# Mingqj/DFU3D

Hardware: AMD Instinct MI355X
Metric: pseudo-box frames/sec (34k pts, 6 cams) (higher is better)
Workload: dtype f64; 1 GPU; configs[1] with depth back-projection on (dense): 64 synthetic frames/GPU/step, 34720-pt sweep, 6 cams x 1600x900 depth + 8 instance masks (one bit-packed 1-byte word per pixel), 30-40 objects/scene; views_per_launch_chunk=192, streams=2, parallelism=frames sharded x1

## Files before the change

dfu3d_amd/csrc/common.hpp:

```cpp
#pragma once
#include <hip/hip_runtime.h>
#include <stdint.h>

#include <stddef.h>
#include <string.h>
#include "dfu3d.h"
#include "dbg.hpp"

#define DFU3D_WAVE 64

struct ViewCalib {
  float M43[12];
  float P2[12];
  float cu, cv, fu, fv, tx, ty;
  float Minv[12];
  float pad[6];
};
static_assert(sizeof(ViewCalib) == DFU3D_CALIB_FLOATS * 4, "calib record");

__device__ __forceinline__ int lane_id() { return threadIdx.x & 63; }

__device__ __forceinline__ int wave_rank(bool flag, int &wave_total) {
  const unsigned long long m = __ballot(flag);
  wave_total = __popcll(m);
  return __popcll(m & ((1ull << lane_id()) - 1ull));
}

template <int NW>
__device__ __forceinline__ int block_rank(bool flag, int *s_w, int &block_total) {
  int wt;
  const int r = wave_rank(flag, wt);
  const int w = threadIdx.x >> 6;
// ... 327 lines not shown
```

dfu3d_amd/csrc/fit_stage.hip:

```cpp
#include "common.hpp"

namespace {
__device__ __forceinline__ int rl_i(int v, int l) { return __builtin_amdgcn_readlane(v, l); }
__device__ __forceinline__ double rl_d(double v, int l) {
  return __hiloint2double(__builtin_amdgcn_readlane(__double2hiint(v), l), __builtin_amdgcn_readlane(__double2loint(v), l));
}

constexpr int CT = 512;
constexpr int GRP = 32;
constexpr int BLK = 32;
constexpr int PAIR_SMALL = 32;
constexpr int GU = 4;
constexpr int SMALL_N = 4096;
constexpr int LARGE_N = 61440;
constexpr int LARGE_GRP = LARGE_N / GRP;
constexpr int GRID_NC_SMALL = 4096;
constexpr int GRID_NC_LARGE = 12288;

struct ParI {
  int *p;
  bool global;
  __device__ __forceinline__ int load(int i) const {
    return __hip_atomic_load(p + i, __ATOMIC_RELAXED, __HIP_MEMORY_SCOPE_AGENT);
  }
// ... 376 lines not shown
  while (true) {
    a = cell_find(par, a);
    b = cell_find(par, b);
    if (a == b) return;
    if (a < b) { const int t = a; a = b; b = t; }
    const int old = atomicMin(par + a, b);
    if (old == a) return;
    a = old;
  }
}

constexpr int CL_CLASSES = 3, CL_TOP = 8192;
template <int NC, int NC_MIN, int TCT>
__global__ __launch_bounds__(TCT, (NC <= GRID_NC_SMALL ? 8 : 4)) void k_range_cluster_grid(
    const double *__restrict__ px, const double *__restrict__ py,
    const long long *__restrict__ seg_base, const int *__restrict__ seg_cnt, double R0,
    double Rd, int *__restrict__ label, double *__restrict__ sx, double *__restrict__ sy,
    int *__restrict__ perm_all, long long pool_cap, int n_lo, int n_hi) {
  __shared__ int s_end[NC];
  __shared__ int s_par[NC];
  __shared__ int s_min[NC];
  __shared__ double s_red[5 * (TCT / 64)];
  __shared__ int s_w[TCT / 64];
  constexpr int NCLS = CL_CLASSES;
  const int S_ = (int)(gridDim.x / (unsigned)NCLS);
  const int cls = (int)(blockIdx.x / (unsigned)S_);
  const int s = (int)(blockIdx.x - (unsigned)cls * (unsigned)S_);
  const int n = seg_cnt[s];
  if (n <= n_lo || n > n_hi) return;
  {
    int mine = NCLS - 1;
#pragma unroll
    for (int k = NCLS - 2; k >= 0; k--) if (n > (CL_TOP >> k)) mine = k;
    if (mine != cls) return;
  }
  const long long base = seg_base[s];
  const double *X = px + base, *Y = py + base;
  double *SX = sx + base, *SY = sy + base;
  int *perm = perm_all + base;
  int *mark = perm_all + 2 * pool_cap + base;
  if (NC_MIN > 0 && *mark) return;
  const GridGeom<NC> G = grid_geometry<NC, TCT>(X, Y, n, R0, Rd, s_red);
  if (threadIdx.x == 0 && (NC_MIN == 0 || G.ok)) *mark = G.ok ? 1 : 0;
  if (!G.ok) return;
  const int ncell = G.ncell;
  for (int c = threadIdx.x; c < ncell; c += TCT) { s_end[c] = 0; s_par[c] = c; s_min[c] = 0x7FFFFFFF; }
// ... 223 lines not shown
#pragma unroll
    for (int u = 0; u < GU; u++) {
      const int i = i0 + u * TCT;
      xs[u] = (i < n) ? SX[i] : 0.0; ys[u] = (i < n) ? SY[i] : 0.0; pm[u] = (i < n) ? perm[i] : 0;
    }
#pragma unroll
    for (int u = 0; u < GU; u++)
      if (i0 + u * TCT < n) glabel[pm[u]] = s_min[cell_find(s_par, grid_cell(G, xs[u], ys[u]))];
  }
}

__global__ __launch_bounds__(CT) void k_range_cluster_fallback(
    const double *__restrict__ px, const double *__restrict__ py,
    const long long *__restrict__ seg_base, const int *__restrict__ seg_cnt, double R0,
    double Rd, int *__restrict__ label, double *__restrict__ sx, double *__restrict__ sy,
    int *__restrict__ si, long long pool_cap) {
  __shared__ __attribute__((aligned(16))) unsigned short s_parent[LARGE_N];
  __shared__ int s_summ[LARGE_GRP];
  __shared__ float4 s_box[LARGE_GRP];
  __shared__ int s_summ2[LARGE_GRP / BLK];
  __shared__ float4 s_box2[LARGE_GRP / BLK];
  __shared__ double s_red[4 * (CT / 64)];
  __shared__ int s_w[CT / 64];
  static_assert(sizeof(int) * SMALL_N <= sizeof(unsigned short) * LARGE_N && SMALL_N / GRP <= LARGE_GRP, "the small form fits");
  const int s = blockIdx.x;
  const int n = seg_cnt[s];
  if (n == 0) return;
  const long long base = seg_base[s];
  if (si[2 * pool_cap + base]) return;
  if (n <= SMALL_N) {
    cell_sort<SMALL_N>(px + base, py + base, n, (int *)s_parent, s_red, s_w, sx + base, sy + base, si + base);
    ParI par{(int *)s_parent, false};
    cluster_body<ParI, SMALL_N / GRP>(par, s_summ, s_box, s_summ2, s_box2, s_red, sx + base, sy + base,
                                      n, R0, Rd, si + base, si + pool_cap + base, label + base);
    return;
  }
  cell_sort<LARGE_N / 2>(px + base, py + base, n, (int *)s_parent, s_red, s_w, sx + base, sy + base,
                         si + base);
  if (n <= LARGE_N) {
    ParH par{s_parent};
    cluster_body<ParH, LARGE_GRP>(par, s_summ, s_box, s_summ2, s_box2, s_red, sx + base, sy + base,
                                  n, R0, Rd, si + base, si + pool_cap + base, label + base);
  } else {
    ParI par{si + 2 * pool_cap + base, true};
    cluster_body<ParI, LARGE_GRP>(par, s_summ, s_box, s_summ2, s_box2, s_red, sx + base, sy + base,
                                  n, R0, Rd, si + base, si + pool_cap + base, label + base);
// ... 95 lines not shown

__device__ __forceinline__ int rank_in(const int *roots, int nk, int L) {
  int lo = 0, hi = nk - 1;
  while (lo < hi) {
    const int mid = (lo + hi) >> 1;
    if (roots[mid] < L) lo = mid + 1; else hi = mid;
  }
  return (roots[lo] == L) ? lo : -1;
}

constexpr int GGU = 4;
__global__ __launch_bounds__(FT) void k_fit_gather(
    const double *__restrict__ px, const double *__restrict__ py,
    const double *__restrict__ pz, const int *__restrict__ label,
    const long long *__restrict__ seg_base, const int *__restrict__ seg_cnt,
    double *__restrict__ gsx, double *__restrict__ gsy, int *__restrict__ sroot,
    uint32_t *__restrict__ status, double *__restrict__ fit_ws, int cap_rows, int cap_big) {
  __shared__ int s_roots[GK];
  __shared__ int s_cnt[FW][GK];
  __shared__ int s_tot[GK], s_off[GK];
  __shared__ double s_red[FW];
  __shared__ int s_w[FW];
  __shared__ int s_q0, s_total;
  const int S_ = (int)(gridDim.x / 3u);
  const int cls = (int)(blockIdx.x / (unsigned)S_);
  const int s = (int)(blockIdx.x - (unsigned)cls * (unsigned)S_);
  const int n = seg_cnt[s];
  if (n == 0) return;
  if (cls != (n > 16384 ? 0 : (n > 8192 ? 1 : 2))) return;
  const long long base = seg_base[s];
  const int wave = threadIdx.x >> 6, lane = lane_id();
  const FitWs W = fit_ws_view(fit_ws, cap_rows, cap_big);

  const int R = (((n + FW - 1) / FW) + 63) & ~63;
  const int r0 = min(n, wave * R), r1 = min(n, r0 + R);
  double zm = -INFINITY;
  int mine = 0;
  for (int c = r0; c < r1; c += 64 * GGU) {
    int L[GGU];
    double zz[GGU];
#pragma unroll
    for (int u = 0; u < GGU; u++) {
      const int i = c + u * 64 + lane;
      L[u] = (i < r1) ? label[base + i] : -1;
      zz[u] = (i < r1) ? pz[base + i] : -INFINITY;
    }
// ... 319 lines not shown
  e.wave_reduce();
  if (lane_id() == 0) { s_ext[wave][0] = e.a0; s_ext[wave][1] = e.a1; s_ext[wave][2] = e.b0; s_ext[wave][3] = e.b1; }
  __syncthreads();
  if (threadIdx.x == 0) {
    double c1min = s_ext[0][0], c1max = s_ext[0][1], c2min = s_ext[0][2], c2max = s_ext[0][3];
    for (int w = 1; w < FW; w++) {
      c1min = fmin(c1min, s_ext[w][0]); c1max = fmax(c1max, s_ext[w][1]);
      c2min = fmin(c2min, s_ext[w][2]); c2max = fmax(c2max, s_ext[w][3]);
    }
    const int s = (int)dsc[0], kc = (int)dsc[1], root = (int)dsc[2];
    const int v = s / max_inst, jinst = s - v * max_inst;
    emit_box(thb, sin_s, cos_s, c1min, c1max, c2min, c2max, dsc[5], s, v, jinst, kc, root, m, calib, inst_class,
             inst_is_car, inst_box, inst_score, car_aspect_max, cap_rows, rows, n_rows, status);
  }
}

__global__ __launch_bounds__(256) void k_fit_tiny(
    const double *__restrict__ gsx, const double *__restrict__ gsy, int max_inst,
    const ViewCalib *__restrict__ calib, const int *__restrict__ inst_class,
    const int *__restrict__ inst_is_car, const float *__restrict__ inst_box,
    const float *__restrict__ inst_score, int n_theta, double dtheta, double car_aspect_max,
    int cap_rows, double *__restrict__ rows, int *__restrict__ n_rows,
    uint32_t *__restrict__ status, double *__restrict__ fit_ws, int cap_big) {
  const FitWs W = fit_ws_view(fit_ws, cap_rows, cap_big);
  const int nq = min(W.counters[0], W.cap_q);
  const int lane = lane_id();
  const int gw = (blockIdx.x * 256 + threadIdx.x) >> 6, nw = (gridDim.x * 256) >> 6;
  for (int e = gw; e < nq; e += nw) {
    const double *d = W.dsc + (size_t)8 * e;
    const int m = (int)d[3];
    if (m > 64) continue;
    const long long P = (long long)d[4];
    const double x = (lane < m) ? gsx[P + lane] : 0.0, y = (lane < m) ? gsy[P + lane] : 0.0;
    const LanePoints pts{x, y, m};
    constexpr int TH_PER_LANE = MAXTH / 64;
    double c1t[TH_PER_LANE], magmax = 0.0, top = -INFINITY;
#pragma unroll
    for (int k = 0; k < TH_PER_LANE; k++) {
      const int th = lane + 64 * k;
      c1t[k] = -INFINITY;
      if (64 * k >= n_theta) continue;
      const double theta = (double)th * dtheta;
      const double ct = cos(theta), st = sin(theta);
      Extent ext;
      ext.clear();
      pts.each([&](double xj, double yj) {
// ... 181 lines not shown
    }
#pragma unroll
    for (int h = 0; h < BIGC_HPW; h++) {
      A[h].wave_reduce();
      double mag;
      const double cst = A[h].cost(mag);
      if (lane == 0 && th[h] < n_theta) {
        W.big_cost[(size_t)c * MAXTH + th[h]] = cst;
        if (mag > 0.0) atomicMax((unsigned long long *)(W.dsc + (size_t)8 * W.big_list[c] + 7), (unsigned long long)__double_as_longlong(mag));
      }
    }
  }
}

__global__ __launch_bounds__(FT) void k_fit_big_box(
    const double *__restrict__ gsx, const double *__restrict__ gsy, int max_inst,
    const ViewCalib *__restrict__ calib, const int *__restrict__ inst_class,
    const int *__restrict__ inst_is_car, const float *__restrict__ inst_box,
    const float *__restrict__ inst_score, int n_theta, double dtheta, double car_aspect_max,
    int cap_rows, double *__restrict__ rows, int *__restrict__ n_rows,
    uint32_t *__restrict__ status, double *__restrict__ fit_ws, int cap_big) {
  __shared__ double s_ext[FW][4];
  __shared__ double s_ct[MAXTH], s_st[MAXTH];
  const FitWs W = fit_ws_view(fit_ws, cap_rows, cap_big);
  const int nbig = min(W.counters[1], cap_big);
  fill_heading_table(s_ct, s_st, dtheta);
  for (int c = blockIdx.x; c < nbig; c += gridDim.x) {
    __syncthreads();
    const double *dsc = W.dsc + (size_t)8 * W.big_list[c];
    const int m = (int)dsc[3];
    const double *mx = gsx + (long long)dsc[4], *my = gsy + (long long)dsc[4];
    const int best = wave_pick_heading(W.big_cost + (size_t)c * MAXTH, n_theta, dsc[7], mx, my, m, s_ct, s_st);
    fit_finish(mx, my, m, dsc, best, dtheta, s_ext, max_inst, calib, inst_class, inst_is_car, inst_box, inst_score,
               car_aspect_max, cap_rows, rows, n_rows, status);
  }
}

}

extern "C" int dfu3d_range_cluster(const double *px, const double *py, const int64_t *seg_base,
                                   const int32_t *seg_cnt, int32_t S, double R0, double Rd,
                                   int32_t *label, double *sx, double *sy, int32_t *si,
                                   int64_t pool_cap, void *stream) {
  DFU3D_CLEAR_STALE_ERROR();
  if (!px || !py || !seg_base || !seg_cnt || !label || !sx || !sy || !si) return DFU3D_EINVAL;
  if (S <= 0 || pool_cap <= 0 || !(R0 > 0.0) || !(Rd >= 0.0)) return DFU3D_EINVAL;
// ... 84 lines not shown
```

dfu3d_amd/csrc/lidar_stage.hip:

```cpp
#include "common.hpp"

namespace {

constexpr int NT = 512;
constexpr int NW = NT / 64;

constexpr int FOV_PW = 1024;
__global__ __launch_bounds__(NT) void k_fov_filter(
    const float4 *__restrict__ pts, const int *__restrict__ pt_off,
    const int *__restrict__ view_frame, const ViewCalib *__restrict__ calib,
    float fovH, float fovW, int capN, int *__restrict__ fov_idx,
    int *__restrict__ n_fov) {
  __shared__ int s_w[NW];
  const int v = blockIdx.x;
  const int f = view_frame[v];
  const int p0 = pt_off[f];
  const int n = pt_off[f + 1] - p0;
  const ViewCalib c = calib[v];
  const int wave = threadIdx.x >> 6, lane = lane_id();
  int running = 0;
  for (int base = 0; base < n; base += NW * FOV_PW) {
    const int w0 = base + wave * FOV_PW;
    unsigned long long flags[FOV_PW / 64];
    int mine = 0;
#pragma unroll
    for (int k = 0; k < FOV_PW / 64; k++) {
      const int i = w0 + k * 64 + lane;
      bool ok = false;
      if (i < n) {
        const float4 p = pts[p0 + i];
        float r[3], u, w, d;
        lidar_to_rect_f32(c.M43, p.x, p.y, p.z, r);
        rect_to_img_f32(c.P2, r, u, w, d);
        ok = (u >= 0.0f) && (u < fovW) && (w >= 0.0f) && (w < fovH) && (d >= 0.0f);
      }
      flags[k] = __ballot(ok);
// ... 147 lines not shown
  return t;
}
__device__ __forceinline__ int block_sum_i(int v, int *s_red) {
  v = wave_sum_i(v);
  const int w = threadIdx.x >> 6;
  __syncthreads();
  if (lane_id() == 0) s_red[w] = v;
  __syncthreads();
  int t = 0;
#pragma unroll
  for (int i = 0; i < NW; i++) t += s_red[i];
  return t;
}

constexpr int RB = 8;
constexpr int RS_LDS = 3072;

__global__ __launch_bounds__(NT) void k_plane_ransac(
    const float4 *__restrict__ pts, const int *__restrict__ pt_off,
    const int *__restrict__ view_frame, const int *__restrict__ fov_idx,
    const int *__restrict__ n_fov, int capN, float max_hs, float xy_range,
    int trials, unsigned long long seed, const long long *__restrict__ key,
    int *__restrict__ cand_idx, double *__restrict__ plane) {
  __shared__ int s_w[NW];
  __shared__ int s_hist[256];
  __shared__ unsigned long long s_sel[3];
  __shared__ double s_red[NW];
  __shared__ int s_redi[NW];
  __shared__ double s_model[RB][3];
  __shared__ int s_valid[RB], s_tot[RB], s_cnt[NW][RB];
  __shared__ float4 s_pt[RS_LDS];
  const int v = blockIdx.x;
  const int p0 = pt_off[view_frame[v]];
  const int nf = n_fov[v];
  const int *fidx = fov_idx + (size_t)v * capN;
  int *cidx = cand_idx + (size_t)v * capN;
  int n = 0;
  for (int base = 0; base < nf; base += NT) {
    const int t = base + threadIdx.x;
    bool ok = false;
    int pi = 0;
    if (t < nf) {
      pi = fidx[t];
      const float4 p = pts[p0 + pi];
      ok = (p.z < max_hs) && (p.x > -xy_range) && (p.x < xy_range) &&
           (p.y > -xy_range) && (p.y < xy_range);
// ... 120 lines not shown
    const double det2 = sxx * syy - sxy * sxy;
    const double ref = fmax(sxx * syy, 1e-300);
    if (det2 > 1e-12 * ref) {
      ca = (sxz * syy - syz * sxy) / det2;
      cb = (syz * sxx - sxz * sxy) / det2;
      cc = (mz - ca * mx) - cb * my;
    }
    const double norm = sqrt((ca * ca + cb * cb) + 1.0);
    out[0] = -(ca / norm);
    out[1] = -(cb / norm);
    out[2] = 1.0 / norm;
    out[3] = -(cc / norm);
  }
}

__global__ __launch_bounds__(NT) void k_project_rows(
    const float4 *__restrict__ pts, const int *__restrict__ pt_off,
    const int *__restrict__ view_frame, const ViewCalib *__restrict__ calib,
    const double *__restrict__ plane, const int *__restrict__ fov_idx,
    const int *__restrict__ n_fov, int capN, float boundH, float boundW, int W,
    double plane_offset, float xy_range, int *__restrict__ ag_pt,
    int *__restrict__ ib_pix, int *__restrict__ n_ag, int *__restrict__ Kout) {
  __shared__ int s_w[NW];
  const int v = blockIdx.x;
  const int p0 = pt_off[view_frame[v]];
  const int nf = n_fov[v];
  const ViewCalib c = calib[v];
  const double pl0 = plane[v * 4 + 0], pl1 = plane[v * 4 + 1], pl2 = plane[v * 4 + 2],
               pl3 = plane[v * 4 + 3];
  const double pn = sqrt((pl0 * pl0 + pl1 * pl1) + pl2 * pl2);
  const int *fidx = fov_idx + (size_t)v * capN;
  int nag = 0, nib = 0;
  for (int base = 0; base < nf; base += NT) {
    const int t = base + threadIdx.x;
    bool ag = false, ib = false;
    int pi = 0, pix = 0;
    if (t < nf) {
      pi = fidx[t];
      const float4 p = pts[p0 + pi];
      double d = (((double)p.x * pl0 + (double)p.y * pl1) + (double)p.z * pl2) + pl3;
      d = d / pn;
      const bool below = d < plane_offset;
      const bool inr = (p.x < xy_range) && (p.x > -xy_range) && (p.y < xy_range) && (p.y > -xy_range);
      ag = !(below && inr);
      if (ag) {
        float r[3], u, w, dep;
// ... 153 lines not shown
```

dfu3d_amd/csrc/segment_stage.hip:

```cpp
#include "common.hpp"

namespace {

constexpr int QT = 256;
constexpr int PT = 1024;

__device__ __forceinline__ uint32_t shadow_word(int seg, double radius) {
  float rf = (float)radius;
  if (radius > 0.0 && (double)rf > radius) rf = __uint_as_float(__float_as_uint(rf) - 1u);
  uint32_t hi = __float_as_uint(rf) >> 16;
  if (radius > 0.0 && hi == 0u) hi = 1u;
  if (radius != radius) hi = 0x7FC0u;
  return ((uint32_t)seg << 16) | hi;
}


constexpr int SEG_WI = 256, SEG_STEPS = SEG_WI / 64;
constexpr int SEG_WPB = 4;
constexpr int SEG_GX = 128;
static_assert(DFU3D_MAX_INST == 32, "one lane per instance, instance bits in one 32-bit word; k_seg_scan: 32 x 32 threads");
inline int seg_ranges(int cap_item) { return (cap_item + SEG_WI - 1) / SEG_WI; }

__device__ __forceinline__ uint32_t wave_or_u32(uint32_t x) { return wave_or_u32_dpp(x); }

// ... 12 lines not shown
  return mine;
}

__global__ __launch_bounds__(SEG_WPB * 64) void k_seg_count(const uint32_t *__restrict__ bits,
                                                            const int *__restrict__ n_item, int cap_item, int NR,
                                                            int *__restrict__ range_cnt) {
  const int v = blockIdx.y;
  const int lane = lane_id();
  const int wave = __builtin_amdgcn_readfirstlane((int)(threadIdx.x >> 6));
  const int n = min(n_item[v], cap_item);
  const int nr = (n + SEG_WI - 1) / SEG_WI;
  for (int r = blockIdx.x * SEG_WPB + wave; r < nr; r += gridDim.x * SEG_WPB) {
    uint32_t b[SEG_STEPS], wany[SEG_STEPS];
#pragma unroll
    for (int k = 0; k < SEG_STEPS; k++) {
      const int t = r * SEG_WI + k * 64 + lane;
      b[k] = (t < n) ? bits[(size_t)v * cap_item + t] : 0u;
    }
    const int mine = wave_instance_counts(b, wany);
    if (lane < DFU3D_MAX_INST) range_cnt[((size_t)v * NR + r) * DFU3D_MAX_INST + lane] = mine;
  }
}

struct SegSide {
  const int *n_item;
  int cap_item, NR;
  int *range_cnt, *cnt;
};
__global__ __launch_bounds__(1024) void k_seg_scan(SegSide A, SegSide B, int max_inst) {
  __shared__ int s_g[32][DFU3D_MAX_INST + 1];
  const SegSide X = blockIdx.y ? B : A;
  const int v = blockIdx.x;
  const int j = threadIdx.x & (DFU3D_MAX_INST - 1), g = threadIdx.x / DFU3D_MAX_INST;
  const int n = min(X.n_item[v], X.cap_item);
  const int nr = (n + SEG_WI - 1) / SEG_WI;
  const int per = (nr + 31) / 32;
  int *col = X.range_cnt + (size_t)v * X.NR * DFU3D_MAX_INST + j;
  const int r0 = g * per, r1 = min(r0 + per, nr);
  int sum = 0;
  for (int r = r0; r < r1; r++) sum += col[(size_t)r * DFU3D_MAX_INST];
  s_g[g][j] = sum;
  __syncthreads();
  int run = 0, tot = 0;
#pragma unroll 8
  for (int q = 0; q < 32; q++) {
    const int c = s_g[q][j];
    run += (q < g) ? c : 0;
    tot += c;
  }
  for (int r = r0; r < r1; r++) {
    const int c = col[(size_t)r * DFU3D_MAX_INST];
    col[(size_t)r * DFU3D_MAX_INST] = run;
    run += c;
  }
  if (g == 0 && j < max_inst) X.cnt[v * max_inst + j] = tot;
}

struct JointSegs {
  long long *base;
  int *cnt;
  double *rad;
  const double *rad_a, *rad_b;
};

__global__ __launch_bounds__(1024) void k_seg_alloc(int S, int *__restrict__ cnt_a,
                                                    int *__restrict__ cnt_b,
                                                    long long *__restrict__ base_a,
                                                    long long *__restrict__ base_b,
                                                    long long pool_cap,
                                                    long long *__restrict__ cursor,
                                                    uint32_t *__restrict__ status, JointSegs J) {
  __shared__ int s_w[16];
  __shared__ long long s_end;
  long long running = *cursor;
  bool over = false;
  if (threadIdx.x == 0) s_end = -1;
  __syncthreads();
  for (int b0 = 0; b0 < S; b0 += 1024) {
    const int s = b0 + threadIdx.x;
    const int ca = (s < S) ? cnt_a[s] : 0, cb = (s < S) ? cnt_b[s] : 0;
    int tot;
    const int ex = block_excl_scan<16>(ca + cb, s_w, tot);
    if (s < S) {
      const long long b = running + ex;
      if (b + ca + cb > pool_cap) {
        cnt_a[s] = 0;
        cnt_b[s] = 0;
        base_a[s] = 0;
        base_b[s] = 0;
        if (ca + cb > 0) {
          over = true;
          atomicMin((unsigned long long *)&s_end, (unsigned long long)b);
        }
      } else {
        base_a[s] = b;
        base_b[s] = b + ca;
      }
      if (J.base) {
        J.base[s] = base_a[s]; J.base[S + s] = base_b[s];
        J.cnt[s] = cnt_a[s]; J.cnt[S + s] = cnt_b[s];
        J.rad[s] = J.rad_a[s]; J.rad[S + s] = J.rad_b[s];
      }
    }
    running += tot;
  }
  if (over) atomicOr(status, DFU3D_ST_POOL_OVERFLOW);
  __syncthreads();
// ... 45 lines not shown
      for (uint32_t w = wany[k]; w; w &= w - 1u) {
        const int j = __ffs((int)w) - 1;
        const bool has = (b[k] >> j) & 1u;
        const unsigned long long m = __ballot(has);
        const long long start = (long long)(((unsigned long long)(uint32_t)__builtin_amdgcn_readlane((int)(woff >> 32), j) << 32) |
                                            (uint32_t)__builtin_amdgcn_readlane((int)(woff & 0xFFFFFFFFll), j));
        const uint32_t swj = (uint32_t)__builtin_amdgcn_readlane((int)sw, j);
        if (has) {
          const long long d = start + __popcll(m & ((1ull << lane) - 1ull));
          px[d] = x[k];
          py[d] = y[k];
          pz[d] = z[k];
          if (pq)
            pq[d] = make_float4((float)x[k], (float)y[k], (float)z[k], __uint_as_float(swj));
        }
        if (lane == j) woff += __popcll(m);
      }
    }
  }
}

template <class F>
__device__ __forceinline__ void tile_scan(int S, F tiles, int *__restrict__ tile_off) {
  __shared__ int s_w[16];
  const int total = block_scan_range<1024, 1, int, int>(S, tiles, [&](int s, int ex) { tile_off[s] = ex; }, s_w);
  if (threadIdx.x == 0) tile_off[S] = total;
}

__global__ __launch_bounds__(1024) void k_tile_scan(int S, const int *__restrict__ cnt,
                                                    int *__restrict__ tile_off, int qt) {
  tile_scan(S, [&](int s) { return (cnt[s] + qt - 1) / qt; }, tile_off);
}

__device__ __forceinline__ int find_segment(const int *tile_off, int S, int t) {
  int lo = 0, hi = S;
  while (hi - lo > 1) {
    const int mid = (lo + hi) >> 1;
    if (tile_off[mid] <= t) lo = mid; else hi = mid;
  }
  return lo;
}

constexpr int RFB = 256;
constexpr int RF_IT = 8;
constexpr int RF_WG = RFB * RF_IT;
constexpr int RF_STRIDE = 8;
constexpr int RF_OCC = 8;
constexpr int RF_GRID = 8192;
constexpr int RF_WLIST = 128;
constexpr int RF_WIN = 16;
constexpr int RF_PLDS = RF_WLIST + 2 * RF_WIN;
constexpr uint32_t RF_NOSEG = 0xFFFFu;
constexpr int BOX_FLOATS = 16;
// ... 428 lines not shown
    cnt += __popcll(__ballot(hit));
  }
  if (big) {
#pragma unroll
    for (int u = 0; u < RF_UL; u++) {
      const bool b = lane + 64 < un[u];
      o[u] = b ? W.uent[ur[u] * RF_WLIST + 64 + lane] : make_float4(0.f, 0.f, 0.f, 0.f);
      op[u] = b ? W.upos[ur[u] * RF_WLIST + 64 + lane] : 0u;
    }
#pragma unroll
    for (int u = 0; u < RF_UL; u++) {
      const bool hit = (op[u] & RF_INCOH) && __float_as_uint(o[u].w) == Q.wq && rf_within(Q, o[u], (long long)(op[u] & ~RF_INCOH), px, py, pz);
      cnt += __popcll(__ballot(hit));
    }
  }
  return cnt;
}

__global__ __launch_bounds__(256, 5) void k_rf_resolve(
    const double *__restrict__ px, const double *__restrict__ py, const double *__restrict__ pz,
    const float4 *__restrict__ pq, const long long *__restrict__ n_used_ptr, long long n_max,
    const long long *__restrict__ seg_base, const int *__restrict__ seg_cnt, const double *__restrict__ radius,
    int nb, int S, RfScratch W) {
  long long n_used = n_max;
  if (n_used_ptr) { const long long u = *n_used_ptr; n_used = u < n_max ? u : n_max; }
  const int wave = (blockIdx.x * 256 + threadIdx.x) >> 6;
  const int nwaves = (gridDim.x * 256) >> 6;
  const int lane = lane_id();
  const int q_incl = wave_incl_scan((int)min((long long)max(W.queue[16 * lane], 0), W.qcap));
  const int nq = __builtin_amdgcn_readlane(q_incl, 63);
  int *lq_tab = W.work + RF_WORK_LQ, *items = W.work + RF_WORK_ITEMS;
  for (int e = wave; e < nq; e += nwaves) {
    const int part = __popcll(__ballot(q_incl <= e));
    const int before = part ? __builtin_amdgcn_readlane(q_incl, part - 1) : 0;
    RfQuery Q;
    if (!rf_load_query(Q, W.queue[RF_QHDR + part * W.qcap + (e - before)], n_max, pq, px, py, pz, seg_base, seg_cnt, radius, S)) continue;
    const int n = (int)(Q.end - Q.base);
    int cnt = 0, n_items = 0, lq = -1;
    if (n <= RF_DIRECT) {
      const long long c_lo = Q.base >> 6, c_hi = (Q.end - 1) >> 6;
      for (long long c0 = c_lo; c0 <= c_hi && cnt <= nb; c0 += RF_SC) {
        float4 o[RF_SC];
#pragma unroll
        for (int u = 0; u < RF_SC; u++) o[u] = pq[((c0 + u) << 6) + lane];
#pragma unroll
        for (int u = 0; u < RF_SC; u++) {
// ... 120 lines not shown
      if ((int)(old >> 32) + 1 == total) W.flags[Q.i] = ((int)(old & 0xFFFFFFFFull) + hits > nb) ? 1 : 0;
    }
  }
}


__global__ __launch_bounds__(QT) void k_shadow_build(
    const double *__restrict__ px, const double *__restrict__ py, const double *__restrict__ pz,
    const long long *__restrict__ seg_base, const int *__restrict__ seg_cnt,
    const double *__restrict__ radius, int S, const int *__restrict__ tile_off, float4 *__restrict__ pq) {
  const int ntile = tile_off[S];
  for (int t = blockIdx.x; t < ntile; t += gridDim.x) {
    const int s = find_segment(tile_off, S, t);
    const int q = (t - tile_off[s]) * QT + threadIdx.x;
    if (q >= seg_cnt[s]) continue;
    const long long i = seg_base[s] + q;
    pq[i] = make_float4((float)px[i], (float)py[i], (float)pz[i], __uint_as_float(shadow_word(s, radius[s])));
  }
}

constexpr int BT_BIG = 1024, BH_HEADS_BIG = 8192, BH_MAX_BIG = 4096;
constexpr int BT_SMALL = 256, BH_HEADS_SMALL = 2048, BH_MAX_SMALL = 1024;

__global__ __launch_bounds__(1024) void k_tile_scan_class(int S, const int *__restrict__ cnt, const int *__restrict__ cnt_a,
                                                          int lo, int hi, int *__restrict__ tile_off, int qt) {
  tile_scan(S, [&](int s) {
    const int na = cnt_a[s];
    return (na > lo && na <= hi) ? (cnt[s] + qt - 1) / qt : 0;
  }, tile_off);
}

__device__ __forceinline__ uint32_t sad_u32(uint32_t a, uint32_t b) {
  uint32_t r;
  asm("v_sad_u32 %0, %1, %2, 0" : "=v"(r) : "v"(a), "v"(b));
  return r;
}
__device__ __forceinline__ uint32_t bh_hash(uint32_t ix, uint32_t iy, uint32_t iz) {
  uint32_t h = __umul24(ix, 0x9E3779u) ^ __umul24(iy, 0x85EBCBu) ^ __umul24(iz, 0xC2B2AFu);
  h ^= h >> 15;
  h ^= h >> 7;
  return h;
}

constexpr int BALL_TPW = 1;
template <int BT, int BH_MAX, int BH_HEADS>
__global__ __launch_bounds__(BT) void k_ball_flags(
    const double *__restrict__ px, const double *__restrict__ py,
    const double *__restrict__ pz, const long long *__restrict__ base_a,
// ... 161 lines not shown
          double d = dx * dx;
          d += dy * dy;
          d += dz * dz;
          if (d < T) { found = true; break; }
        }
        if (!found) s_pending = 1;
      }
      __syncthreads();
      if (!s_pending && any_kept) break;
    }
    if (valid && any_kept) flags[bq + q] = found ? 1 : 0;
  }
}


constexpr int CPT = 1024;
constexpr int CPE = 2;
__global__ __launch_bounds__(CPT) void k_seg_compact(
    double *__restrict__ px, double *__restrict__ py, double *__restrict__ pz,
    long long *__restrict__ seg_base, int *__restrict__ seg_cnt,
    const uint8_t *__restrict__ flags, const long long *__restrict__ dst_after_base,
    int *__restrict__ dst_after_cnt, int compact_front) {
  __shared__ int s_w[CPT / 64];
  const int s = blockIdx.x;
  const int n = seg_cnt[s];
  const long long src = seg_base[s];
  const int front_all = dst_after_base ? dst_after_cnt[s] : 0;
  const int front = (compact_front && dst_after_base) ? front_all : 0;
  const long long src_f = dst_after_base ? dst_after_base[s] : 0;
  const long long dst = dst_after_base ? src_f + (front_all - front) : src;
  const int n_all = front + n;
  if (n_all == 0) {
    if (dst_after_base && threadIdx.x == 0) seg_base[s] = dst;
    return;
  }
  int running = 0, kept_front = 0;
  for (int t0 = 0; t0 < n_all; t0 += CPT * CPE) {
    const int i0 = t0 + threadIdx.x * CPE;
    bool f[CPE];
    double x[CPE], y[CPE], z[CPE];
    int mine = 0;
#pragma unroll
    for (int k = 0; k < CPE; k++) {
      const int i = i0 + k;
      const long long g = (i < front) ? src_f + i : src + (i - front);
      f[k] = (i < n_all) && flags[g];
// ... 249 lines not shown
    double *pz, int64_t *base_a, int32_t *cnt_a, int64_t *base_b, int32_t *cnt_b,
    uint32_t *status, const double *rad_a, const double *rad_b, void *shadow, int64_t *base_ab,
    int32_t *cnt_ab, double *rad_ab, int32_t *chunk_cnt, void *stream) {
  DFU3D_CLEAR_STALE_ERROR();
  if (!a_bits || !a_x || !a_y || !a_z || !a_n || !b_bits || !b_x || !b_y || !b_z || !b_n ||
      !pool_cursor || !px || !py || !pz || !base_a || !cnt_a || !base_b || !cnt_b || !status || !chunk_cnt)
    return DFU3D_EINVAL;
  if (V <= 0 || max_inst <= 0 || a_cap <= 0 || b_cap <= 0 || pool_cap <= 0) return DFU3D_EINVAL;
  if (max_inst > DFU3D_MAX_INST) return DFU3D_ERANGE;
  if ((shadow || base_ab) && (!rad_a || !rad_b)) return DFU3D_EINVAL;
  if (base_ab && (!cnt_ab || !rad_ab)) return DFU3D_EINVAL;
  const int S = V * max_inst;
  if (shadow && 2 * (int64_t)S >= (int64_t)RF_NOSEG) return DFU3D_ERANGE;
  if (shadow && ((uintptr_t)shadow & 15u)) return DFU3D_EINVAL;
  hipStream_t st = (hipStream_t)stream;
  const int nra = seg_ranges(a_cap), nrb = seg_ranges(b_cap);
  int32_t *rc_a = chunk_cnt, *rc_b = chunk_cnt + seg_count_words(V, a_cap);
  const int gxa = std::min((nra + SEG_WPB - 1) / SEG_WPB, SEG_GX), gxb = std::min((nrb + SEG_WPB - 1) / SEG_WPB, SEG_GX);
  hipLaunchKernelGGL(k_seg_count, dim3(gxa, V), dim3(SEG_WPB * 64), 0, st, a_bits, a_n, a_cap, nra, rc_a);
  DFU3D_LAUNCH_CHECK();
  hipLaunchKernelGGL(k_seg_count, dim3(gxb, V), dim3(SEG_WPB * 64), 0, st, b_bits, b_n, b_cap, nrb, rc_b);
  DFU3D_LAUNCH_CHECK();
  const SegSide SA = {a_n, a_cap, nra, rc_a, cnt_a}, SB = {b_n, b_cap, nrb, rc_b, cnt_b};
  hipLaunchKernelGGL(k_seg_scan, dim3(V, 2), dim3(1024), 0, st, SA, SB, max_inst);
  DFU3D_LAUNCH_CHECK();
  const JointSegs J = {(long long *)base_ab, cnt_ab, rad_ab, rad_a, rad_b};
  hipLaunchKernelGGL(k_seg_alloc, dim3(1), dim3(1024), 0, st, S, cnt_a, cnt_b,
                     (long long *)base_a, (long long *)base_b, (long long)pool_cap,
                     (long long *)pool_cursor, status, J);
  DFU3D_LAUNCH_CHECK();
  hipLaunchKernelGGL(k_seg_write, dim3(gxa, (V + 7) / 8 * 8), dim3(SEG_WPB * 64), 0, st, a_bits, a_x, a_y, a_z, a_n, a_cap,
                     max_inst, nra, (const long long *)base_a, cnt_a, rc_a, px, py, pz, (float4 *)shadow, rad_a, 0, V);
  DFU3D_LAUNCH_CHECK();
  hipLaunchKernelGGL(k_seg_write, dim3(gxb, (V + 7) / 8 * 8), dim3(SEG_WPB * 64), 0, st, b_bits, b_x, b_y, b_z, b_n, b_cap,
                     max_inst, nrb, (const long long *)base_b, cnt_b, rc_b, px, py, pz, (float4 *)shadow, rad_b, S, V);
  DFU3D_LAUNCH_CHECK();
  return DFU3D_OK;
}

extern "C" int64_t dfu3d_rf_shadow_bytes(int64_t pool_cap) { return pool_cap > 0 ? DFU3D_SHADOW_BYTES(pool_cap) : DFU3D_EINVAL; }
extern "C" int64_t dfu3d_rf_queue_ints(int64_t pool_cap) { return pool_cap > 0 ? DFU3D_RF_QUEUE_INTS(pool_cap) : DFU3D_EINVAL; }

extern "C" int dfu3d_radius_filter(double *px, double *py, double *pz, const int64_t *seg_base,
                                   int32_t *seg_cnt, const double *radius, int32_t nb_points,
                                   int32_t S, int64_t pool_cap, const int64_t *n_used, void *shadow,
                                   int32_t *tile_off, uint8_t *flags, int32_t *queue, int32_t phases,
                                   void *stream) {
  DFU3D_CLEAR_STALE_ERROR();
  if (!px || !py || !pz || !seg_base || !seg_cnt || !radius || !tile_off || !flags || !queue || !shadow)
    return DFU3D_EINVAL;
  if (S <= 0 || pool_cap <= 0 || nb_points < 0) return DFU3D_EINVAL;
  if (pool_cap >= (1ll << 31) - 2) return DFU3D_ERANGE;
  if ((int64_t)S >= (int64_t)RF_NOSEG) return DFU3D_ERANGE;
  if ((uintptr_t)shadow & 15u) return DFU3D_EINVAL;
  hipStream_t st = (hipStream_t)stream;
  const RfCut C = rf_cut(shadow, pool_cap);
  if (C.bytes > DFU3D_SHADOW_BYTES(pool_cap) || RF_QHDR + RF_QSHARDS * (int64_t)C.W.qcap > DFU3D_RF_QUEUE_INTS(pool_cap))
    return DFU3D_ERANGE;
  float4 *pq = C.pq;
  const int64_t n_ranges = C.n_ranges;
  RfScratch W = C.W;
  W.flags = flags;
  W.queue = queue;
  W.seg_base = (const long long *)seg_base;
  if (phases & DFU3D_RF_SHADOW) {
    if (dfu3d_fill_async(pq, 0xFF, sizeof(float4) * (size_t)pool_cap, st) != hipSuccess) return DFU3D_ELAUNCH;
    hipLaunchKernelGGL(k_tile_scan, dim3(1), dim3(1024), 0, st, S, seg_cnt, tile_off, QT);
    DFU3D_LAUNCH_CHECK();
    const int g = tile_grid(pool_cap, S);
    hipLaunchKernelGGL(k_shadow_build, dim3(g < 4096 ? g : 4096), dim3(QT), 0, st, px, py, pz,
                       (const long long *)seg_base, seg_cnt, radius, S, tile_off, pq);
    DFU3D_LAUNCH_CHECK();
  }
  if (phases & DFU3D_RF_FLAGS) {
    if (dfu3d_fill_small_async(queue, RF_QHDR * sizeof(int), W.work, sizeof(int) * (size_t)(RF_WORK_HDR + S), nullptr, 0, st) != hipSuccess)
      return DFU3D_ELAUNCH;
    const long long n_tiles = (pool_cap + RF_WG - 1) / RF_WG;
    const dim3 grid((unsigned)(n_tiles < RF_GRID ? n_tiles : RF_GRID));
    if (nb_points == 1)
      hipLaunchKernelGGL(k_rf_stream<true>, grid, dim3(RFB), 0, st, pq, (const long long *)n_used, (long long)pool_cap,
                         nb_points, S, W);
    else
      hipLaunchKernelGGL(k_rf_stream<false>, grid, dim3(RFB), 0, st, pq, (const long long *)n_used, (long long)pool_cap,
                         nb_points, S, W);
    DFU3D_LAUNCH_CHECK();
    const long long g_pair = ((long long)n_ranges + 3) / 4;
    hipLaunchKernelGGL(k_rf_pair, dim3((unsigned)(g_pair < 4096 ? g_pair : 4096)), dim3(256), 0, st, (const long long *)n_used,
                       (long long)pool_cap, nb_points, W);
    DFU3D_LAUNCH_CHECK();
  }
// ... 25 lines not shown
  DFU3D_CLEAR_STALE_ERROR();
  if (!px || !py || !pz || !seg_base || !seg_cnt || !enable || !scratch || !status) return DFU3D_EINVAL;
  if (S <= 0 || pool_cap <= 0 || !(voxel_size > 0.0) || !(voxel_size < 1e300)) return DFU3D_EINVAL;
  if (pool_cap >= (1ll << 29)) return DFU3D_ERANGE;
  if ((uintptr_t)scratch & 7u) return DFU3D_EINVAL;
  hipLaunchKernelGGL(k_voxel_down, dim3(S), dim3(VD_T), 0, (hipStream_t)stream, px, py, pz, (const long long *)seg_base,
                     seg_cnt, enable, voxel_size, vd_scratch(scratch, pool_cap), status);
  DFU3D_LAUNCH_CHECK();
  return DFU3D_OK;
}

extern "C" int dfu3d_stat_filter(double *px, double *py, double *pz, const int64_t *seg_base,
                                 int32_t *seg_cnt, const int32_t *enable, int32_t nb_neighbors,
                                 double std_ratio, int32_t S, int64_t pool_cap,
                                 int32_t *tile_off, uint8_t *flags, double *mean_d,
                                 double *stats, void *stream) {
  DFU3D_CLEAR_STALE_ERROR();
  (void)stats;
  if (!px || !py || !pz || !seg_base || !seg_cnt || !enable || !tile_off || !flags || !mean_d)
    return DFU3D_EINVAL;
  if (S <= 0 || pool_cap <= 0 || nb_neighbors < 1) return DFU3D_EINVAL;
  if (nb_neighbors > KMAX) return DFU3D_ERANGE;
  hipStream_t st = (hipStream_t)stream;
  hipLaunchKernelGGL(k_tile_scan, dim3(1), dim3(1024), 0, st, S, seg_cnt, tile_off, KQ);
  DFU3D_LAUNCH_CHECK();
  if (hipFuncSetAttribute((const void *)k_knn_mean, hipFuncAttributeMaxDynamicSharedMemorySize, (int)(sizeof(double) * KMAX * KQ)) != hipSuccess)
    return DFU3D_ELAUNCH;
  hipLaunchKernelGGL(k_knn_mean, dim3((unsigned)((pool_cap + KQ - 1) / KQ + S)), dim3(KQ), sizeof(double) * (size_t)nb_neighbors * KQ, st,
                     px, py, pz, (const long long *)seg_base, seg_cnt, enable, nb_neighbors, S, tile_off,
                     mean_d);
  DFU3D_LAUNCH_CHECK();
  hipLaunchKernelGGL(k_stat_flags, dim3(S), dim3(256), 0, st, (const long long *)seg_base,
                     seg_cnt, enable, std_ratio, mean_d, flags);
  DFU3D_LAUNCH_CHECK();
  hipLaunchKernelGGL(k_seg_compact, dim3(S), dim3(CPT), 0, st, px, py, pz,
                     (long long *)seg_base, seg_cnt, flags, (const long long *)nullptr,
                     (int *)nullptr, 0);
  DFU3D_LAUNCH_CHECK();
  return DFU3D_OK;
}

static int ballquery_fuse_impl(double *px, double *py, double *pz, const int64_t *base_a,
                                    int32_t *cnt_a, int64_t *base_b, int32_t *cnt_b,
                                    double C, int32_t S, int64_t pool_cap, int32_t *tile_off,
                                    uint8_t *flags, int masked, void *stream) {
  DFU3D_CLEAR_STALE_ERROR();
  if (!px || !py || !pz || !base_a || !cnt_a || !base_b || !cnt_b || !tile_off || !flags)
    return DFU3D_EINVAL;
  if (S <= 0 || pool_cap <= 0) return DFU3D_EINVAL;
  if (!(C > 0.0) || !(C < 1e150)) return DFU3D_EINVAL;
  hipStream_t st = (hipStream_t)stream;
  double T = C * C;
  while (__builtin_sqrt(T) >= C) T = __builtin_nextafter(T, 0.0);
  while (__builtin_sqrt(T) < C) T = __builtin_nextafter(T, __builtin_inf());
  int32_t *tile_small = tile_off, *tile_big = tile_off + S + 1;
  hipLaunchKernelGGL(k_tile_scan_class, dim3(1), dim3(1024), 0, st, S, cnt_b, cnt_a, -1, BH_MAX_SMALL, tile_small, BT_SMALL);
  DFU3D_LAUNCH_CHECK();
  hipLaunchKernelGGL(k_tile_scan_class, dim3(1), dim3(1024), 0, st, S, cnt_b, cnt_a, BH_MAX_SMALL, 0x7FFFFFFF, tile_big, BT_BIG);
  DFU3D_LAUNCH_CHECK();
  const int g_small = (int)(((pool_cap + BT_SMALL - 1) / BT_SMALL + S + BALL_TPW - 1) / BALL_TPW);
  hipLaunchKernelGGL((k_ball_flags<BT_SMALL, BH_MAX_SMALL, BH_HEADS_SMALL>), dim3(g_small), dim3(BT_SMALL), 0, st, px, py, pz,
                     (const long long *)base_a, cnt_a, (const long long *)base_b, cnt_b, T, C, S,
                     tile_small, flags, masked);
  DFU3D_LAUNCH_CHECK();
  const int g_big = (int)(((pool_cap + BT_BIG - 1) / BT_BIG + S + BALL_TPW - 1) / BALL_TPW);
  hipLaunchKernelGGL((k_ball_flags<BT_BIG, BH_MAX_BIG, BH_HEADS_BIG>), dim3(g_big), dim3(BT_BIG), 0, st, px, py, pz,
                     (const long long *)base_a, cnt_a, (const long long *)base_b, cnt_b, T, C, S,
                     tile_big, flags, masked);
  DFU3D_LAUNCH_CHECK();
  hipLaunchKernelGGL(k_seg_compact, dim3(S), dim3(CPT), 0, st, px, py, pz, (long long *)base_b,
                     cnt_b, flags, (const long long *)base_a, cnt_a, masked == 2 ? 1 : 0);
  DFU3D_LAUNCH_CHECK();
  return DFU3D_OK;
}

extern "C" int dfu3d_ballquery_fuse(double *px, double *py, double *pz, const int64_t *base_a,
                                    const int32_t *cnt_a, int64_t *base_b, int32_t *cnt_b,
                                    double C, int32_t S, int64_t pool_cap, int32_t *tile_off,
                                    uint8_t *flags, void *stream) {
  return ballquery_fuse_impl(px, py, pz, base_a, (int32_t *)cnt_a, base_b, cnt_b, C, S, pool_cap, tile_off,
                             flags, 0, stream);
// ... 20 lines not shown
```

Baseline: 10540 frames/s.

## Raise wave priority on tail kernels and shrink single-block scans to 256 threads

Adds a macro that calls s_setprio in many small or serial tail kernels (clustering, fit, lidar, segment scans, compaction). With two streams in flight, these kernels should then win instruction issue over the bulk work running beside them. The single-block scan kernels (seg_scan, seg_alloc, tile_scan) also drop from 1024 to 256 threads, each thread handling 4 consecutive items, which shortens the barrier and wave-scan cost on the critical path. The risk is that the bulk kernels running in parallel get starved, and that per-thread serial work in the scans grows.

```diff
diff --git a/dfu3d_amd/csrc/common.hpp b/dfu3d_amd/csrc/common.hpp
--- a/dfu3d_amd/csrc/common.hpp
+++ b/dfu3d_amd/csrc/common.hpp
@@ -8,6 +8,11 @@
 #include "dbg.hpp"
 
 #define DFU3D_WAVE 64
+
+#ifndef DFU3D_TAIL_PRIO
+#define DFU3D_TAIL_PRIO 2
+#endif
+#define DFU3D_RAISE_PRIO() do { if (DFU3D_TAIL_PRIO) __builtin_amdgcn_s_setprio(DFU3D_TAIL_PRIO); } while (0)
 
 struct ViewCalib {
   float M43[12];
diff --git a/dfu3d_amd/csrc/fit_stage.hip b/dfu3d_amd/csrc/fit_stage.hip
--- a/dfu3d_amd/csrc/fit_stage.hip
+++ b/dfu3d_amd/csrc/fit_stage.hip
@@ -422,6 +422,7 @@
   __shared__ int s_min[NC];
   __shared__ double s_red[5 * (TCT / 64)];
   __shared__ int s_w[TCT / 64];
+  DFU3D_RAISE_PRIO();
   constexpr int NCLS = CL_CLASSES;
   const int S_ = (int)(gridDim.x / (unsigned)NCLS);
   const int cls = (int)(blockIdx.x / (unsigned)S_);
@@ -691,6 +692,7 @@
   __shared__ float4 s_box2[LARGE_GRP / BLK];
   __shared__ double s_red[4 * (CT / 64)];
   __shared__ int s_w[CT / 64];
+  DFU3D_RAISE_PRIO();
   static_assert(sizeof(int) * SMALL_N <= sizeof(unsigned short) * LARGE_N && SMALL_N / GRP <= LARGE_GRP, "the small form fits");
   const int s = blockIdx.x;
   const int n = seg_cnt[s];
@@ -832,6 +834,7 @@
   __shared__ double s_red[FW];
   __shared__ int s_w[FW];
   __shared__ int s_q0, s_total;
+  DFU3D_RAISE_PRIO();
   const int S_ = (int)(gridDim.x / 3u);
   const int cls = (int)(blockIdx.x / (unsigned)S_);
   const int s = (int)(blockIdx.x - (unsigned)cls * (unsigned)S_);
@@ -1197,6 +1200,7 @@
     const float *__restrict__ inst_score, int n_theta, double dtheta, double car_aspect_max,
     int cap_rows, double *__restrict__ rows, int *__restrict__ n_rows,
     uint32_t *__restrict__ status, double *__restrict__ fit_ws, int cap_big) {
+  DFU3D_RAISE_PRIO();
   const FitWs W = fit_ws_view(fit_ws, cap_rows, cap_big);
   const int nq = min(W.counters[0], W.cap_q);
   const int lane = lane_id();
@@ -1424,6 +1428,7 @@
     uint32_t *__restrict__ status, double *__restrict__ fit_ws, int cap_big) {
   __shared__ double s_ext[FW][4];
   __shared__ double s_ct[MAXTH], s_st[MAXTH];
+  DFU3D_RAISE_PRIO();
   const FitWs W = fit_ws_view(fit_ws, cap_rows, cap_big);
   const int nbig = min(W.counters[1], cap_big);
   fill_heading_table(s_ct, s_st, dtheta);
diff --git a/dfu3d_amd/csrc/lidar_stage.hip b/dfu3d_amd/csrc/lidar_stage.hip
--- a/dfu3d_amd/csrc/lidar_stage.hip
+++ b/dfu3d_amd/csrc/lidar_stage.hip
@@ -12,6 +12,7 @@
     float fovH, float fovW, int capN, int *__restrict__ fov_idx,
     int *__restrict__ n_fov) {
   __shared__ int s_w[NW];
+  DFU3D_RAISE_PRIO();
   const int v = blockIdx.x;
   const int f = view_frame[v];
   const int p0 = pt_off[f];
@@ -205,6 +206,7 @@
     const int *__restrict__ n_fov, int capN, float max_hs, float xy_range,
     int trials, unsigned long long seed, const long long *__restrict__ key,
     int *__restrict__ cand_idx, double *__restrict__ plane) {
+  DFU3D_RAISE_PRIO();
   __shared__ int s_w[NW];
   __shared__ int s_hist[256];
   __shared__ unsigned long long s_sel[3];
@@ -371,6 +373,7 @@
     double plane_offset, float xy_range, int *__restrict__ ag_pt,
     int *__restrict__ ib_pix, int *__restrict__ n_ag, int *__restrict__ Kout) {
   __shared__ int s_w[NW];
+  DFU3D_RAISE_PRIO();
   const int v = blockIdx.x;
   const int p0 = pt_off[view_frame[v]];
   const int nf = n_fov[v];
diff --git a/dfu3d_amd/csrc/segment_stage.hip b/dfu3d_amd/csrc/segment_stage.hip
--- a/dfu3d_amd/csrc/segment_stage.hip
+++ b/dfu3d_amd/csrc/segment_stage.hip
@@ -58,13 +58,17 @@
   }
 }
 
+constexpr int SCAN_T = 256;
+constexpr int SCAN_K = 4;
+static_assert(SCAN_T / DFU3D_MAX_INST * SCAN_K == 32, "k_seg_scan: 32 row groups per column");
 struct SegSide {
   const int *n_item;
   int cap_item, NR;
   int *range_cnt, *cnt;
 };
-__global__ __launch_bounds__(1024) void k_seg_scan(SegSide A, SegSide B, int max_inst) {
+__global__ __launch_bounds__(SCAN_T) void k_seg_scan(SegSide A, SegSide B, int max_inst) {
   __shared__ int s_g[32][DFU3D_MAX_INST + 1];
+  DFU3D_RAISE_PRIO();
   const SegSide X = blockIdx.y ? B : A;
   const int v = blockIdx.x;
   const int j = threadIdx.x & (DFU3D_MAX_INST - 1), g = threadIdx.x / DFU3D_MAX_INST;
@@ -72,22 +76,42 @@
   const int nr = (n + SEG_WI - 1) / SEG_WI;
   const int per = (nr + 31) / 32;
   int *col = X.range_cnt + (size_t)v * X.NR * DFU3D_MAX_INST + j;
-  const int r0 = g * per, r1 = min(r0 + per, nr);
-  int sum = 0;
-  for (int r = r0; r < r1; r++) sum += col[(size_t)r * DFU3D_MAX_INST];
-  s_g[g][j] = sum;
+  int sum[SCAN_K];
+#pragma unroll
+  for (int k = 0; k < SCAN_K; k++) sum[k] = 0;
+  for (int i = 0; i < per; i++) {
+#pragma unroll
+    for (int k = 0; k < SCAN_K; k++) {
+      const int r = (g * SCAN_K + k) * per + i;
+      sum[k] += (r < nr) ? col[(size_t)r * DFU3D_MAX_INST] : 0;
+    }
+  }
+#pragma unroll
+  for (int k = 0; k < SCAN_K; k++) s_g[g * SCAN_K + k][j] = sum[k];
   __syncthreads();
-  int run = 0, tot = 0;
+  int before = 0, tot = 0;
 #pragma unroll 8
   for (int q = 0; q < 32; q++) {
     const int c = s_g[q][j];
-    run += (q < g) ? c : 0;
+    before += (q < g * SCAN_K) ? c : 0;
     tot += c;
   }
-  for (int r = r0; r < r1; r++) {
-    const int c = col[(size_t)r * DFU3D_MAX_INST];
-    col[(size_t)r * DFU3D_MAX_INST] = run;
-    run += c;
+  int run[SCAN_K];
+#pragma unroll
+  for (int k = 0; k < SCAN_K; k++) {
+    run[k] = before;
+    before += sum[k];
+  }
+  for (int i = 0; i < per; i++) {
+#pragma unroll
+    for (int k = 0; k < SCAN_K; k++) {
+      const int r = (g * SCAN_K + k) * per + i;
+      if (r < nr) {
+        const int c = col[(size_t)r * DFU3D_MAX_INST];
+        col[(size_t)r * DFU3D_MAX_INST] = run[k];
+        run[k] += c;
+      }
+    }
   }
   if (g == 0 && j < max_inst) X.cnt[v * max_inst + j] = tot;
 }
@@ -99,26 +123,37 @@
   const double *rad_a, *rad_b;
 };
 
-__global__ __launch_bounds__(1024) void k_seg_alloc(int S, int *__restrict__ cnt_a,
+__global__ __launch_bounds__(SCAN_T) void k_seg_alloc(int S, int *__restrict__ cnt_a,
                                                     int *__restrict__ cnt_b,
                                                     long long *__restrict__ base_a,
                                                     long long *__restrict__ base_b,
                                                     long long pool_cap,
                                                     long long *__restrict__ cursor,
                                                     uint32_t *__restrict__ status, JointSegs J) {
-  __shared__ int s_w[16];
+  __shared__ int s_w[SCAN_T / 64];
   __shared__ long long s_end;
+  DFU3D_RAISE_PRIO();
   long long running = *cursor;
   bool over = false;
   if (threadIdx.x == 0) s_end = -1;
   __syncthreads();
-  for (int b0 = 0; b0 < S; b0 += 1024) {
-    const int s = b0 + threadIdx.x;
-    const int ca = (s < S) ? cnt_a[s] : 0, cb = (s < S) ? cnt_b[s] : 0;
+  for (int b0 = 0; b0 < S; b0 += SCAN_T * SCAN_K) {
+    const int s0 = b0 + (int)threadIdx.x * SCAN_K;
+    int cak[SCAN_K], cbk[SCAN_K], mine = 0;
+#pragma unroll
+    for (int k = 0; k < SCAN_K; k++) {
+      cak[k] = (s0 + k < S) ? cnt_a[s0 + k] : 0;
+      cbk[k] = (s0 + k < S) ? cnt_b[s0 + k] : 0;
+      mine += cak[k] + cbk[k];
+    }
     int tot;
-    const int ex = block_excl_scan<16>(ca + cb, s_w, tot);
-    if (s < S) {
+    int ex = block_excl_scan<SCAN_T / 64>(mine, s_w, tot);
+#pragma unroll
+    for (int k = 0; k < SCAN_K; k++) {
+      const int s = s0 + k, ca = cak[k], cb = cbk[k];
+      if (s >= S) break;
       const long long b = running + ex;
+      ex += ca + cb;
       if (b + ca + cb > pool_cap) {
         cnt_a[s] = 0;
         cnt_b[s] = 0;
@@ -210,13 +245,14 @@
 
 template <class F>
 __device__ __forceinline__ void tile_scan(int S, F tiles, int *__restrict__ tile_off) {
-  __shared__ int s_w[16];
-  const int total = block_scan_range<1024, 1, int, int>(S, tiles, [&](int s, int ex) { tile_off[s] = ex; }, s_w);
+  __shared__ int s_w[SCAN_T / 64];
+  DFU3D_RAISE_PRIO();
+  const int total = block_scan_range<SCAN_T, SCAN_K, int, int>(S, tiles, [&](int s, int ex) { tile_off[s] = ex; }, s_w);
   if (threadIdx.x == 0) tile_off[S] = total;
 }
 
-__global__ __launch_bounds__(1024) void k_tile_scan(int S, const int *__restrict__ cnt,
-                                                    int *__restrict__ tile_off, int qt) {
+__global__ __launch_bounds__(SCAN_T) void k_tile_scan(int S, const int *__restrict__ cnt,
+                                                      int *__restrict__ tile_off, int qt) {
   tile_scan(S, [&](int s) { return (cnt[s] + qt - 1) / qt; }, tile_off);
 }
 
@@ -691,6 +727,7 @@
     const float4 *__restrict__ pq, const long long *__restrict__ n_used_ptr, long long n_max,
     const long long *__restrict__ seg_base, const int *__restrict__ seg_cnt, const double *__restrict__ radius,
     int nb, int S, RfScratch W) {
+  DFU3D_RAISE_PRIO();
   long long n_used = n_max;
   if (n_used_ptr) { const long long u = *n_used_ptr; n_used = u < n_max ? u : n_max; }
   const int wave = (blockIdx.x * 256 + threadIdx.x) >> 6;
@@ -857,8 +894,8 @@
 constexpr int BT_BIG = 1024, BH_HEADS_BIG = 8192, BH_MAX_BIG = 4096;
 constexpr int BT_SMALL = 256, BH_HEADS_SMALL = 2048, BH_MAX_SMALL = 1024;
 
-__global__ __launch_bounds__(1024) void k_tile_scan_class(int S, const int *__restrict__ cnt, const int *__restrict__ cnt_a,
-                                                          int lo, int hi, int *__restrict__ tile_off, int qt) {
+__global__ __launch_bounds__(SCAN_T) void k_tile_scan_class(int S, const int *__restrict__ cnt, const int *__restrict__ cnt_a,
+                                                            int lo, int hi, int *__restrict__ tile_off, int qt) {
   tile_scan(S, [&](int s) {
     const int na = cnt_a[s];
     return (na > lo && na <= hi) ? (cnt[s] + qt - 1) / qt : 0;
@@ -1066,6 +1103,7 @@
     const uint8_t *__restrict__ flags, const long long *__restrict__ dst_after_base,
     int *__restrict__ dst_after_cnt, int compact_front) {
   __shared__ int s_w[CPT / 64];
+  DFU3D_RAISE_PRIO();
   const int s = blockIdx.x;
   const int n = seg_cnt[s];
   const long long src = seg_base[s];
@@ -1361,10 +1399,10 @@
   hipLaunchKernelGGL(k_seg_count, dim3(gxb, V), dim3(SEG_WPB * 64), 0, st, b_bits, b_n, b_cap, nrb, rc_b);
   DFU3D_LAUNCH_CHECK();
   const SegSide SA = {a_n, a_cap, nra, rc_a, cnt_a}, SB = {b_n, b_cap, nrb, rc_b, cnt_b};
-  hipLaunchKernelGGL(k_seg_scan, dim3(V, 2), dim3(1024), 0, st, SA, SB, max_inst);
+  hipLaunchKernelGGL(k_seg_scan, dim3(V, 2), dim3(SCAN_T), 0, st, SA, SB, max_inst);
   DFU3D_LAUNCH_CHECK();
   const JointSegs J = {(long long *)base_ab, cnt_ab, rad_ab, rad_a, rad_b};
-  hipLaunchKernelGGL(k_seg_alloc, dim3(1), dim3(1024), 0, st, S, cnt_a, cnt_b,
+  hipLaunchKernelGGL(k_seg_alloc, dim3(1), dim3(SCAN_T), 0, st, S, cnt_a, cnt_b,
                      (long long *)base_a, (long long *)base_b, (long long)pool_cap,
                      (long long *)pool_cursor, status, J);
   DFU3D_LAUNCH_CHECK();
@@ -1404,7 +1442,7 @@
   W.seg_base = (const long long *)seg_base;
   if (phases & DFU3D_RF_SHADOW) {
     if (dfu3d_fill_async(pq, 0xFF, sizeof(float4) * (size_t)pool_cap, st) != hipSuccess) return DFU3D_ELAUNCH;
-    hipLaunchKernelGGL(k_tile_scan, dim3(1), dim3(1024), 0, st, S, seg_cnt, tile_off, QT);
+    hipLaunchKernelGGL(k_tile_scan, dim3(1), dim3(SCAN_T), 0, st, S, seg_cnt, tile_off, QT);
     DFU3D_LAUNCH_CHECK();
     const int g = tile_grid(pool_cap, S);
     hipLaunchKernelGGL(k_shadow_build, dim3(g < 4096 ? g : 4096), dim3(QT), 0, st, px, py, pz,
@@ -1476,7 +1514,7 @@
   if (S <= 0 || pool_cap <= 0 || nb_neighbors < 1) return DFU3D_EINVAL;
   if (nb_neighbors > KMAX) return DFU3D_ERANGE;
   hipStream_t st = (hipStream_t)stream;
-  hipLaunchKernelGGL(k_tile_scan, dim3(1), dim3(1024), 0, st, S, seg_cnt, tile_off, KQ);
+  hipLaunchKernelGGL(k_tile_scan, dim3(1), dim3(SCAN_T), 0, st, S, seg_cnt, tile_off, KQ);
   DFU3D_LAUNCH_CHECK();
   if (hipFuncSetAttribute((const void *)k_knn_mean, hipFuncAttributeMaxDynamicSharedMemorySize, (int)(sizeof(double) * KMAX * KQ)) != hipSuccess)
     return DFU3D_ELAUNCH;
@@ -1508,9 +1546,9 @@
   while (__builtin_sqrt(T) >= C) T = __builtin_nextafter(T, 0.0);
   while (__builtin_sqrt(T) < C) T = __builtin_nextafter(T, __builtin_inf());
   int32_t *tile_small = tile_off, *tile_big = tile_off + S + 1;
-  hipLaunchKernelGGL(k_tile_scan_class, dim3(1), dim3(1024), 0, st, S, cnt_b, cnt_a, -1, BH_MAX_SMALL, tile_small, BT_SMALL);
+  hipLaunchKernelGGL(k_tile_scan_class, dim3(1), dim3(SCAN_T), 0, st, S, cnt_b, cnt_a, -1, BH_MAX_SMALL, tile_small, BT_SMALL);
   DFU3D_LAUNCH_CHECK();
-  hipLaunchKernelGGL(k_tile_scan_class, dim3(1), dim3(1024), 0, st, S, cnt_b, cnt_a, BH_MAX_SMALL, 0x7FFFFFFF, tile_big, BT_BIG);
+  hipLaunchKernelGGL(k_tile_scan_class, dim3(1), dim3(SCAN_T), 0, st, S, cnt_b, cnt_a, BH_MAX_SMALL, 0x7FFFFFFF, tile_big, BT_BIG);
   DFU3D_LAUNCH_CHECK();
   const int g_small = (int)(((pool_cap + BT_SMALL - 1) / BT_SMALL + S + BALL_TPW - 1) / BALL_TPW);
   hipLaunchKernelGGL((k_ball_flags<BT_SMALL, BH_MAX_SMALL, BH_HEADS_SMALL>), dim3(g_small), dim3(BT_SMALL), 0, st, px, py, pz,
```

Measured after the change: 10570 frames/s (median of 6 runs). Within noise of the previous version (+0.2%).
